# lhoyer/improving_segmentation_with_selfsupervised_depth

Hardware: AMD Instinct MI355X
Metric: train images/sec, ResNet-101 joint seg+depth @512x1024 (higher is better)
Workload: dtype f32

## Files before the change

improving_segmentation_with_selfsupervised_depth_amd/_lib.py:

```python
import ctypes
import os
from ctypes import c_int, c_long, c_float, c_void_p, c_size_t, c_uint64, c_int64, POINTER

_HERE = os.path.dirname(os.path.abspath(__file__))
LIB_PATH = os.environ.get("SEGSDE_LIB") or os.path.join(_HERE, "libsegsde_hip.so")
ABI_VERSION = 15

_LIB = None
HOST_POINTERS_OK = False


class PackJob(ctypes.Structure):
    _fields_ = [("w", c_void_p), ("fwd", c_void_p), ("dgrad", c_void_p)] + [(n, c_int) for n in (
        "O", "I", "KH", "KW", "block0", "reserved")]


class WinoJob(ctypes.Structure):
    _fields_ = [("w", c_void_p), ("u_fwd", c_void_p), ("u_dgrad", c_void_p)] + [(n, c_int) for n in ("O", "I", "block0", "reserved")]


class ConvDesc(ctypes.Structure):
    _fields_ = [(n, c_int) for n in (
        "B", "H", "W", "C0", "C1", "ld0", "ld1", "up0", "Ho", "Wo", "Cout", "ldy", "ldy2", "nsplit",
        "KH", "KW", "stride", "dil", "pad", "pad_mode", "in_div", "act", "sum2x2", "accumulate", "compute")]


P = c_void_p
_SIGS = {
    "segsde_abi_version": (c_int, []),
    "segsde_conv_compute_taken": (c_int, [POINTER(ConvDesc), c_int]),
    "segsde_split_bf16_planes": (c_int, [P, c_long, P, P, P, P]),
    "segsde_conv2d_forward": (c_int, [POINTER(ConvDesc), P, P, P, P, P, P, P]),
    "segsde_conv2d_stats_rows": (c_long, [POINTER(ConvDesc)]),
    "segsde_conv2d_forward_stats": (c_int, [POINTER(ConvDesc), P, P, P, P, P, P, P, P]),
    "segsde_conv2d_dgrad_actgrad": (c_int, [POINTER(ConvDesc), P, P, P, P, P, P, P, P, c_int, c_int, P]),
    "segsde_bn_stats_from_partials_workspace": (c_size_t, [c_int]),
    "segsde_bn_stats_from_partials": (c_int, [P, c_long, c_long, c_int, P, P, P, P, c_float, c_float, P, P, c_size_t, P]),
    "segsde_conv2d_wgrad_workspace": (c_size_t, [POINTER(ConvDesc)]),
    "segsde_conv2d_wgrad": (c_int, [POINTER(ConvDesc), P, P, P, c_int, P, P, c_size_t, P]),
# ... 5 lines not shown
    "segsde_conv2d_wgrad_winograd_workspace": (c_size_t, [POINTER(ConvDesc)]),
    "segsde_conv2d_wgrad_winograd": (c_int, [POINTER(ConvDesc), P, P, P, c_int, P, P, P, c_size_t, P]),
    "segsde_winograd_fused_ok": (c_int, [c_int, c_int, c_int, c_int, c_int]),
    "segsde_winograd_fused_stats_rows": (ctypes.c_long, [c_int, c_int, c_int]),
    "segsde_winograd_fused_pack": (c_int, [P, c_int, c_int, c_int, P, P]),
    "segsde_conv2d_winograd_fused": (c_int, [P, c_int, c_int, c_int, c_int, c_int, c_int, P, c_int, P, c_int, P, c_int, c_int, P, P]),
    "segsde_conv2d_winograd_fused2": (c_int, [P, c_int, c_int, c_int, P, c_int, c_int, c_int, c_int, c_int, c_int, P, c_int, P, c_int, P,
                                              c_int, P, P]),
    "segsde_conv2d_winograd_fused_dgrad": (c_int, [P, c_int, c_int, c_int, c_int, c_int, P, c_int, c_int, P, c_int, c_int, P, c_int, c_int, P]),
    "segsde_reflect_adjoint_borders": (c_int, [P, P, P, P, P, c_int, c_int, P]),
    "segsde_reflect_adjoint_borders_ok": (c_int, [P, c_int]),
    "segsde_reflect_adjoint_borders2": (c_int, [P, c_int, P, c_int, P, c_int, P, c_int, c_int, c_int, c_int, c_int, c_int, c_int, P]),
    "segsde_conv2d_wgrad_winograd_fused_workspace": (c_size_t, [P]),
    "segsde_conv2d_wgrad_winograd_fused": (c_int, [P, P, P, P, c_int, P, P, c_size_t, P]),
    "segsde_upfold_pack": (c_int, [P, c_int, c_int, c_int, P, P, P]),
    "segsde_conv2d_forward_upfold": (c_int, [POINTER(ConvDesc), P, P, P, P, P, P, P]),
    "segsde_conv2d_dgrad_upfold": (c_int, [POINTER(ConvDesc), P, c_int, P, P, P, P, P, c_int, P, c_int, c_int, P]),
    "segsde_conv2d_wgrad_upfold_workspace": (c_size_t, [POINTER(ConvDesc)]),
    "segsde_conv2d_wgrad_upfold": (c_int, [POINTER(ConvDesc), P, P, P, c_int, P, P, c_size_t, P]),
    "segsde_stem_pack": (c_int, [P, c_int, c_int, c_int, P, P]),
    "segsde_stem7x7_stats_rows": (c_long, [c_int, c_int, c_int, c_int, c_int]),
    "segsde_stem7x7_forward": (c_int, [P, c_int, c_int, c_int, c_int, P, c_int, P, P, P]),
    "segsde_stem7x7_wgrad_workspace": (c_size_t, [c_int, c_int, c_int, c_int, c_int]),
    "segsde_stem7x7_wgrad": (c_int, [P, c_int, c_int, c_int, c_int, P, c_int, c_int, c_int, P, P, c_size_t, P]),
    "segsde_nchw_to_nhwc_bordered": (c_int, [P, c_int, c_int, c_int, c_int, c_float, c_float, P, c_int, c_int, c_int, c_int, c_int, P]),
    "segsde_pack_weight": (c_int, [P, P, c_int, c_int, c_int, c_int, c_int, P]),
    "segsde_pack_weight_both": (c_int, [P, P, P, c_int, c_int, c_int, c_int, P]),
    "segsde_pack_weight_both_multi": (c_int, [P, c_int, c_int, P]),
    "segsde_reflect_dgrad_fix": (c_int, [P, c_int, P, P, c_int, P, c_int, c_int, c_int, c_int, c_int, c_int, c_int, P]),
    "segsde_bn_stats_workspace": (c_size_t, [c_long, c_int]),
    "segsde_bn_stats": (c_int, [P, c_int, c_long, c_int, P, P, P, P, c_float, c_float, P, P, c_size_t, P]),
    "segsde_bn_eval_stats": (c_int, [P, P, c_int, c_float, P, P, P]),
    "segsde_bn_apply": (c_int, [P, c_int, c_long, c_int, P, P, P, P, P, c_int, P, c_int, c_int, c_float, c_uint64, P]),
    "segsde_bn_backward_workspace": (c_size_t, [c_long, c_int]),
    "segsde_bn_backward": (c_int, [P, c_int, P, c_int, P, c_int, c_long, c_int, P, P, P, P, c_int, c_float, c_uint64, c_int,
                                   P, P, P, c_int, P, c_int, P, c_size_t, P]),
    "segsde_colsum_workspace": (c_size_t, [c_long, c_int]),
    "segsde_act_backward": (c_int, [P, c_int, P, c_int, c_long, c_int, c_int, P, c_int, P, P, c_size_t, P]),
    "segsde_colsum": (c_int, [P, c_int, c_long, c_int, P, P, c_size_t, P]),
    "segsde_feat_dist_workspace": (c_size_t, [c_long, c_int]),
    "segsde_feat_dist_forward": (c_int, [P, c_int, P, c_int, c_long, c_int, P, P, c_size_t, P]),
    "segsde_feat_dist_backward": (c_int, [P, c_int, P, c_int, c_long, c_int, P, P, P, c_int, P]),
    "segsde_maxpool3x3s2_forward": (c_int, [P, c_int, c_int, c_int, c_int, P, P, P]),
    "segsde_maxpool3x3s2_backward": (c_int, [P, P, c_int, c_int, c_int, c_int, P, c_int, P]),
    "segsde_upsample2x_backward": (c_int, [P, c_int, c_int, c_int, c_int, c_int, P, c_int, P]),
    "segsde_upsample2x_forward": (c_int, [P, c_int, c_int, c_int, c_int, c_int, P, c_int, P]),
    "segsde_resize_bilinear_forward": (c_int, [P, c_int, c_int, c_int, c_int, c_int, P, c_int, c_int, c_int, c_int, P]),
    "segsde_resize_bilinear_backward": (c_int, [P, c_int, c_int, c_int, c_int, c_int, P, c_int, c_int, c_int, c_int, P]),
    "segsde_global_avgpool_workspace": (c_size_t, [c_int, c_long, c_int]),
    "segsde_global_avgpool_forward": (c_int, [P, c_int, c_int, c_long, c_int, P, P, c_size_t, P]),
    "segsde_global_avgpool_backward": (c_int, [P, c_int, c_long, c_int, P, c_int, P]),
    "segsde_gate_forward": (c_int, [P, P, c_long, P, P]),
    "segsde_gate_backward": (c_int, [P, P, P, c_long, P, P, P]),
    "segsde_axpby": (c_int, [c_long, c_float, P, c_float, P, P, P]),
    "segsde_axpby_dev": (c_int, [c_long, P, P, P, P, P, P]),
    "segsde_scale_channels": (c_int, [P, c_int, c_int, c_long, c_int, P, P, c_int, P]),
    "segsde_dropout": (c_int, [P, c_int, c_long, c_int, c_float, c_uint64, P, c_int, P]),
    "segsde_copy_channels": (c_int, [P, c_int, P, c_int, c_long, c_int, P]),
    "segsde_nchw_to_nhwc": (c_int, [P, c_int, c_int, c_int, c_int, c_float, c_float, P, c_int, P]),
    "segsde_nhwc_to_nchw": (c_int, [P, c_int, c_int, c_int, c_int, c_int, P, P]),
    "segsde_pose_matrix_forward": (c_int, [P, P, c_int, c_int, c_int, P, P]),
    "segsde_pose_matrix_backward": (c_int, [P, P, P, c_int, c_int, c_int, P, P, P]),
    "segsde_warp_forward": (c_int, [P, c_int, c_int, P, P, P, P, c_int, c_int, c_int, c_float, c_float, P, P, P, P]),
    "segsde_warp_backward_workspace": (c_size_t, [c_int, c_int, c_int]),
    "segsde_warp_backward": (c_int, [P, P, c_int, c_int, P, P, P, P, c_int, c_int, c_int, c_float, c_float, P, P, P,
                                     c_size_t, P]),
    "segsde_reprojection_error_forward": (c_int, [P, P, c_int, c_int, c_int, c_int, P, c_long, P]),
# ... 74 lines not shown
```

improving_segmentation_with_selfsupervised_depth_amd/csrc/elementwise.hip:

```cpp
#include <stdlib.h>
#include "segsde_common.h"
#include <type_traits>
#include <utility>
#include <cstdlib>
#include <cstring>

namespace {

template <int VW> struct VecF { float v[VW]; };
template <int VW> __device__ __forceinline__ VecF<VW> ldv(const float* p) {
  VecF<VW> r;
  if (VW == 4) { const float4 t = *reinterpret_cast<const float4*>(p); r.v[0] = t.x; r.v[1 % VW] = t.y; r.v[2 % VW] = t.z; r.v[3 % VW] = t.w; }
  else r.v[0] = p[0];
  return r;
}
template <int VW> __device__ __forceinline__ void stv(float* p, const VecF<VW>& r) {
  if (VW == 4) *reinterpret_cast<float4*>(p) = make_float4(r.v[0], r.v[1 % VW], r.v[2 % VW], r.v[3 % VW]);
  else p[0] = r.v[0];
}

constexpr int SLAB = 64;
constexpr int RLANES = 4;

__host__ __device__ inline int red_blocks(long M) {
// ... 97 lines not shown
                                                                float momentum, float* mean, float* invstd,
                                                                float* running_mean, float* running_var, int64_t* nbt) {
  SEGSDE_SMEM;
  double* sh = reinterpret_cast<double*>(segsde_smem);
  const int c = blockIdx.x * 16 + (threadIdx.x & 15), pl = threadIdx.x >> 4;
  if (nbt && blockIdx.x == 0 && threadIdx.x == 0) nbt[0] += 1;
  double s, q;
  combine_partials(part, nb, C, c, pl, sh, s, q);
  if (pl != 0 || c >= C) return;
  const double mu = s / (double)M;
  double var = q / (double)M - mu * mu;
  if (var < 0.0) var = 0.0;
  mean[c] = (float)mu;
  invstd[c] = (float)(1.0 / sqrt(var + (double)eps));
  if (running_mean) running_mean[c] = (1.f - momentum) * running_mean[c] + momentum * (float)mu;
  if (running_var) {
    const double unb = M > 1 ? var * (double)M / (double)(M - 1) : var;
    running_var[c] = (1.f - momentum) * running_var[c] + momentum * (float)unb;
  }
}

__global__ __launch_bounds__(256) void bn_eval_stats_kernel(const float* rm, const float* rv, int C, float eps,
                                                            float* mean, float* invstd) {
  const int c = blockIdx.x * 256 + threadIdx.x;
  if (c >= C) return;
  mean[c] = rm[c];
  invstd[c] = 1.0f / sqrtf(rv[c] + eps);
}

template <int VW>
__global__ __launch_bounds__(256) void bn_apply_kernel(const float* x, int ldx, long M, int C, const float* mean,
                                                       const float* invstd, const float* gamma, const float* beta,
                                                       const float* res, int ldr, float* y, int ldy, int act,
                                                       float drop_p, uint64_t seed, int cv_shift) {
  const int CV = C / VW;
  const long total = M * CV;
  const float keep_scale = drop_p > 0.f ? 1.f / (1.f - drop_p) : 1.f;
  const long stride = (long)gridDim.x * 256;
  const bool fixed_c = cv_shift >= 0 && (stride & (long)(CV - 1)) == 0;
  VecF<VW> mu, is, ga, be;
  if (fixed_c) {
    const int c = (int)((blockIdx.x * 256L + threadIdx.x) & (long)(CV - 1)) * VW;
    mu = ldv<VW>(mean + c); is = ldv<VW>(invstd + c);
    if (gamma) { ga = ldv<VW>(gamma + c); be = ldv<VW>(beta + c); }
  }
  auto finish = [&](long m, int c, const VecF<VW>& xv, const VecF<VW>& rv) {
    VecF<VW> o;
#pragma unroll
    for (int j = 0; j < VW; ++j) {
      float t = (xv.v[j] - mu.v[j]) * is.v[j];
      if (gamma) t = t * ga.v[j] + be.v[j];
      if (res) t += rv.v[j];
      t = segsde_act(t, act);
      if (drop_p > 0.f) t = segsde_uniform01(seed, (uint64_t)(m * C + c + j)) >= drop_p ? t * keep_scale : 0.f;
      o.v[j] = t;
    }
    stv<VW>(y + m * ldy + c, o);
  };
  long e = blockIdx.x * 256L + threadIdx.x;
  for (; e < total; e += stride) {
    const long m = cv_shift >= 0 ? (e >> cv_shift) : e / CV;
    const int c = (int)(e - m * CV) * VW;
    const VecF<VW> xv = ldv<VW>(x + m * ldx + c);
    if (!fixed_c) {
      mu = ldv<VW>(mean + c); is = ldv<VW>(invstd + c);
      if (gamma) { ga = ldv<VW>(gamma + c); be = ldv<VW>(beta + c); }
    }
    VecF<VW> rv;
    if (res) rv = ldv<VW>(res + m * ldr + c);
    finish(m, c, xv, rv);
  }
}

__device__ __forceinline__ float bn_dz(float dy, float y, int act, float drop_p, uint64_t seed, uint64_t idx) {
  float g = dy;
  if (drop_p > 0.f) {
    const bool keep = segsde_uniform01(seed, idx) >= drop_p;
    if (!keep) return 0.f;
    const float ks = 1.f / (1.f - drop_p);
    g *= ks;
    y = y / ks;
  }
  return g * segsde_act_grad_from_out(y, act);
}

__device__ __forceinline__ float bn_dz_remask(float dy, float xh, float gamma, float beta, bool affine, int act) {
  if (act != SEGSDE_ACT_RELU) return dy;
  float t = xh;
  if (affine) t = t * gamma + beta;
  return t > 0.f ? dy : 0.f;
}

struct BnBwdOp {
  const float* dy; int lddy; const float* y; int ldy; const float* x; int ldx; const float* mean; const float* invstd;
  int act, C; float drop_p; uint64_t seed; const float* gamma; const float* beta;
  template <int VW> struct Ctx { VecF<VW> mu, is, ga, be; };
  template <int VW> __device__ Ctx<VW> ctx(int c) const {
    Ctx<VW> k;
    k.mu = ldv<VW>(mean + c); k.is = ldv<VW>(invstd + c);
    if (!y && gamma) { k.ga = ldv<VW>(gamma + c); k.be = ldv<VW>(beta + c); }
    return k;
  }
  template <int VW> __device__ void row(long m, int c, const Ctx<VW>& k, double* s0, double* s1) const {
    const VecF<VW> g = ldv<VW>(dy + m * lddy + c), xx = ldv<VW>(x + m * ldx + c);
    VecF<VW> yy;
    if (y) yy = ldv<VW>(y + m * ldy + c);
#pragma unroll
    for (int j = 0; j < VW; ++j) {
      const float xh = (xx.v[j] - k.mu.v[j]) * k.is.v[j];
      const float dz = y ? bn_dz(g.v[j], yy.v[j], act, drop_p, seed, (uint64_t)(m * C + c + j))
                         : bn_dz_remask(g.v[j], xh, gamma ? k.ga.v[j] : 1.f, gamma ? k.be.v[j] : 0.f, gamma != nullptr, act);
      s0[j] += (double)dz * (double)xh; s1[j] += (double)dz;
    }
  }
};

__global__ __launch_bounds__(256) void pair_finalize_kernel(const double* part, int nb, int C, float* out0, float* out1) {
  SEGSDE_SMEM;
  double* sh = reinterpret_cast<double*>(segsde_smem);
  const int c = blockIdx.x * 16 + (threadIdx.x & 15), pl = threadIdx.x >> 4;
  double a, b;
  combine_partials(part, nb, C, c, pl, sh, a, b);
  if (pl != 0 || c >= C) return;
  if (out0) out0[c] = (float)a;
  if (out1) out1[c] = (float)b;
}

template <int VW>
__global__ __launch_bounds__(256) void bn_bwd_apply_kernel(const float* dy, int lddy, const float* y, int ldy,
                                                           const float* x, int ldx, long M, int C, const float* mean,
                                                           const float* invstd, const float* gamma, const float* beta,
                                                           int act, float drop_p, uint64_t seed, int batch_stats,
                                                           const float* dgamma, const float* dbeta, float* dx, int lddx,
                                                           float* dres, int lddres, int cv_shift) {
  const int CV = C / VW;
  const long total = M * CV;
  const float invM = 1.f / (float)M;
  const bool remask = y == nullptr;
  const long stride = (long)gridDim.x * 256;
  const bool fixed_c = cv_shift >= 0 && (stride & (long)(CV - 1)) == 0;
  VecF<VW> ga, be, mu, is, dg, db;
  auto load_params = [&](int c) {
    if (dx || remask) {
      is = ldv<VW>(invstd + c);
      if (gamma) ga = ldv<VW>(gamma + c);
      if (gamma && remask) be = ldv<VW>(beta + c);
// ... 1 lines not shown
      if (batch_stats && dx) { dg = ldv<VW>(dgamma + c); db = ldv<VW>(dbeta + c); }
    }
  };
  if (fixed_c) load_params((int)((blockIdx.x * 256L + threadIdx.x) & (long)(CV - 1)) * VW);
  auto finish = [&](long m, int c, const VecF<VW>& g, const VecF<VW>& xx, const VecF<VW>& yy) {
    VecF<VW> dz, o;
#pragma unroll
    for (int j = 0; j < VW; ++j) {
      if (remask) dz.v[j] = bn_dz_remask(g.v[j], (xx.v[j] - mu.v[j]) * is.v[j], gamma ? ga.v[j] : 1.f, gamma ? be.v[j] : 0.f, gamma != nullptr, act);
      else dz.v[j] = bn_dz(g.v[j], yy.v[j], act, drop_p, seed, (uint64_t)(m * C + c + j));
      if (dx) {
        const float gm = gamma ? ga.v[j] : 1.f;
        if (batch_stats) {
          const float xh = (xx.v[j] - mu.v[j]) * is.v[j];
          o.v[j] = gm * is.v[j] * (dz.v[j] - db.v[j] * invM - xh * dg.v[j] * invM);
        } else {
          o.v[j] = gm * is.v[j] * dz.v[j];
        }
      }
    }
    if (dres) stv<VW>(dres + m * lddres + c, dz);
    if (dx) stv<VW>(dx + m * lddx + c, o);
  };
  long e = blockIdx.x * 256L + threadIdx.x;
  for (; e < total; e += stride) {
    const long m = cv_shift >= 0 ? (e >> cv_shift) : e / CV;
    const int c = (int)(e - m * CV) * VW;
    const VecF<VW> g = ldv<VW>(dy + m * lddy + c);
    VecF<VW> xx, yy;
    if (!remask) yy = ldv<VW>(y + m * ldy + c);
    if ((dx && batch_stats) || remask) xx = ldv<VW>(x + m * ldx + c);
    if (!fixed_c) load_params(c);
    finish(m, c, g, xx, yy);
  }
}

struct ActBwdOp {
  const float* dy; int lddy; const float* y; int ldy; float* dz; int lddz; int act;
  template <int VW> __device__ void row(long m, int c, double* s0, double* s1) const {
    const VecF<VW> g = ldv<VW>(dy + m * lddy + c), yy = ldv<VW>(y + m * ldy + c);
    VecF<VW> o;
#pragma unroll
    for (int j = 0; j < VW; ++j) { o.v[j] = g.v[j] * segsde_act_grad_from_out(yy.v[j], act); s0[j] += (double)o.v[j]; }
    if (dz) stv<VW>(dz + m * lddz + c, o);
  }
};
struct ColsumOp {
  const float* x; int ld;
  template <int VW> __device__ void row(long m, int c, double* s0, double* s1) const {
    const VecF<VW> t = ldv<VW>(x + m * ld + c);
#pragma unroll
    for (int j = 0; j < VW; ++j) s0[j] += (double)t.v[j];
  }
};

__global__ __launch_bounds__(256) void maxpool_fwd_kernel(const float* x, int B, int H, int W, int C, int Ho, int Wo,
                                                          float* y, uint8_t* idx) {
  const long total = (long)B * Ho * Wo * C;
  for (long e = blockIdx.x * 256L + threadIdx.x; e < total; e += (long)gridDim.x * 256) {
    const int c = (int)(e % C); long t = e / C;
    const int wo = (int)(t % Wo); t /= Wo;
    const int ho = (int)(t % Ho); const int b = (int)(t / Ho);
    float best = -INFINITY; int bi = 0; bool first = true;
    for (int kh = 0; kh < 3; ++kh) {
      const int h = 2 * ho - 1 + kh;
      if (h < 0 || h >= H) continue;
// ... 478 lines not shown
  if (!partials || !mean || !invstd || !ws) return SEGSDE_ERR_NULL;
  if (rows <= 0 || M <= 0 || C <= 0) return SEGSDE_ERR_SHAPE;
  if (ws_bytes < segsde_bn_stats_from_partials_workspace(C)) return SEGSDE_ERR_WORKSPACE;
  if (rows <= 64) {
    hipLaunchKernelGGL(bn_stats_from_partials_kernel, dim3((C + 15) / 16), dim3(256), 4096, ST(stream), partials, rows, M, C, eps,
                       momentum, mean, invstd, running_mean, running_var, num_batches_tracked);
    SEGSDE_CHECK_LAUNCH();
    return 0;
  }
  if (rows <= partials_wide_max()) {
    hipLaunchKernelGGL(bn_stats_from_partials_wide_kernel, dim3((C + 3) / 4), dim3(256), 4096, ST(stream), partials, rows, M, C, eps,
                       momentum, mean, invstd, running_mean, running_var, num_batches_tracked);
    SEGSDE_CHECK_LAUNCH();
    return 0;
  }
  const int nb = rows < PARTIALS_NB ? (int)rows : PARTIALS_NB;
  hipLaunchKernelGGL(bn_partials_reduce_kernel, dim3(nb, (C + 63) / 64), dim3(256), 4096, ST(stream), partials, rows, C, nb,
                     (double*)ws);
  SEGSDE_CHECK_LAUNCH();
  hipLaunchKernelGGL(bn_stats_finalize_kernel, dim3((C + 15) / 16), dim3(256), 4096, ST(stream), (const double*)ws, nb, M, C,
                     eps, momentum, mean, invstd, running_mean, running_var, num_batches_tracked);
  SEGSDE_CHECK_LAUNCH();
  return 0;
}

extern "C" int segsde_bn_eval_stats(const float* rm, const float* rv, int C, float eps, float* mean, float* invstd,
                                    void* stream) {
  if (!rm || !rv || !mean || !invstd) return SEGSDE_ERR_NULL;
  hipLaunchKernelGGL(bn_eval_stats_kernel, dim3((C + 255) / 256), dim3(256), 0, ST(stream), rm, rv, C, eps, mean, invstd);
  SEGSDE_CHECK_LAUNCH();
  return 0;
}

extern "C" int segsde_bn_apply(const float* x, int ldx, long M, int C, const float* mean, const float* invstd,
                               const float* gamma, const float* beta, const float* residual, int ldr, float* y, int ldy,
                               int act, float drop_p, uint64_t seed, void* stream) {
  if (!x || !mean || !invstd || !y) return SEGSDE_ERR_NULL;
  if ((gamma == nullptr) != (beta == nullptr)) return SEGSDE_ERR_NULL;
  if (M <= 0 || C <= 0 || drop_p < 0.f || drop_p >= 1.f) return SEGSDE_ERR_SHAPE;
  const bool v4 = (C % 4 == 0) && (ldx % 4 == 0) && (ldy % 4 == 0) && al16(x) && al16(y) &&
                  (!residual || ((ldr % 4 == 0) && al16(residual)));
  if (v4)
    hipLaunchKernelGGL(bn_apply_kernel<4>, dim3(ew_blocks_cv(M * C / 4, C / 4)), dim3(256), 0, ST(stream), x, ldx, M, C, mean,
                       invstd, gamma, beta, residual, ldr, y, ldy, act, drop_p, seed, pow2_shift(C / 4));
  else
    hipLaunchKernelGGL(bn_apply_kernel<1>, dim3(ew_blocks_cv(M * C, C)), dim3(256), 0, ST(stream), x, ldx, M, C, mean, invstd,
                       gamma, beta, residual, ldr, y, ldy, act, drop_p, seed, pow2_shift(C));
  SEGSDE_CHECK_LAUNCH();
  return 0;
}

extern "C" int segsde_bn_backward(const float* dy, int lddy, const float* y, int ldy, const float* x, int ldx, long M,
                                  int C, const float* mean, const float* invstd, const float* gamma, const float* beta,
                                  int act, float drop_p, uint64_t seed, int batch_stats, float* dgamma, float* dbeta,
                                  float* dx, int lddx, float* dres, int lddres, void* ws, size_t ws_bytes, void* stream) {
  if (!dy || !x || !mean || !invstd || !dgamma || !dbeta || !ws) return SEGSDE_ERR_NULL;
  if (!y) {
    if (!(act == SEGSDE_ACT_NONE || (act == SEGSDE_ACT_RELU && drop_p <= 0.f && !dres && (!gamma || beta)))) return SEGSDE_ERR_NULL;
  }
  if (M <= 0 || C <= 0) return SEGSDE_ERR_SHAPE;
  if (ws_bytes < part_bytes(M, C)) return SEGSDE_ERR_WORKSPACE;
  if (!y) ldy = ldx;
  BnBwdOp op{dy, lddy, y, ldy, x, ldx, mean, invstd, act, C, drop_p, seed, gamma, beta};
  const bool vec = (C % 4 == 0) && (ldx % 4 == 0) && (ldy % 4 == 0) && (lddy % 4 == 0) && al16p(x) && (!y || al16p(y)) && al16p(dy) &&
                   (!gamma || (al16p(gamma) && (!beta || al16p(beta)))) && al16p(mean) && al16p(invstd);
  if (int e = launch_colreduce(op, M, C, (double*)ws, vec, ST(stream))) return e;
  hipLaunchKernelGGL(pair_finalize_kernel, dim3((C + 15) / 16), dim3(256), 4096, ST(stream), (const double*)ws,
                     red_blocks(M), C, dgamma, dbeta);
  SEGSDE_CHECK_LAUNCH();
  if (dx || dres) {
    const bool v4 = vec && (!dx || ((lddx % 4 == 0) && al16p(dx))) && (!dres || ((lddres % 4 == 0) && al16p(dres))) &&
                    al16p(dgamma) && al16p(dbeta);
    if (v4)
      hipLaunchKernelGGL(bn_bwd_apply_kernel<4>, dim3(ew_blocks_cv(M * C / 4, C / 4)), dim3(256), 0, ST(stream), dy, lddy, y, ldy, x,
                         ldx, M, C, mean, invstd, gamma, beta, act, drop_p, seed, batch_stats, (const float*)dgamma,
                         (const float*)dbeta, dx, lddx, dres, lddres, pow2_shift(C / 4));
    else
      hipLaunchKernelGGL(bn_bwd_apply_kernel<1>, dim3(ew_blocks_cv(M * C, C)), dim3(256), 0, ST(stream), dy, lddy, y, ldy, x, ldx,
                         M, C, mean, invstd, gamma, beta, act, drop_p, seed, batch_stats, (const float*)dgamma,
                         (const float*)dbeta, dx, lddx, dres, lddres, pow2_shift(C));
    SEGSDE_CHECK_LAUNCH();
  }
  return 0;
}

extern "C" int segsde_act_backward(const float* dy, int lddy, const float* y, int ldy, long M, int C, int act, float* dz,
                                   int lddz, float* dbias, void* ws, size_t ws_bytes, void* stream) {
  if (!dy || !y || !ws) return SEGSDE_ERR_NULL;
  if (M <= 0 || C <= 0) return SEGSDE_ERR_SHAPE;
  if (ws_bytes < part_bytes(M, C)) return SEGSDE_ERR_WORKSPACE;
  ActBwdOp op{dy, lddy, y, ldy, dz, lddz, act};
  const bool vec = (C % 4 == 0) && (ldy % 4 == 0) && (lddy % 4 == 0) && al16p(y) && al16p(dy) &&
                   (!dz || ((lddz % 4 == 0) && al16p(dz)));
  if (int e = launch_colreduce(op, M, C, (double*)ws, vec, ST(stream))) return e;
  if (dbias) {
    hipLaunchKernelGGL(pair_finalize_kernel, dim3((C + 15) / 16), dim3(256), 4096, ST(stream), (const double*)ws,
                       red_blocks(M), C, dbias, (float*)nullptr);
    SEGSDE_CHECK_LAUNCH();
  }
  return 0;
}

extern "C" int segsde_colsum(const float* x, int ldx, long M, int C, float* out, void* ws, size_t ws_bytes, void* stream) {
  if (!x || !out || !ws) return SEGSDE_ERR_NULL;
  if (M <= 0 || C <= 0) return SEGSDE_ERR_SHAPE;
  if (ws_bytes < part_bytes(M, C)) return SEGSDE_ERR_WORKSPACE;
  ColsumOp op{x, ldx};
  const bool vec = (C % 4 == 0) && (ldx % 4 == 0) && al16p(x);
  if (int e = launch_colreduce(op, M, C, (double*)ws, vec, ST(stream))) return e;
  hipLaunchKernelGGL(pair_finalize_kernel, dim3((C + 15) / 16), dim3(256), 4096, ST(stream), (const double*)ws,
                     red_blocks(M), C, out, (float*)nullptr);
  SEGSDE_CHECK_LAUNCH();
  return 0;
// ... 188 lines not shown
```

improving_segmentation_with_selfsupervised_depth_amd/functional.py:

```python
import collections
import weakref

import torch
from torch.autograd import Function as _TorchFunction

from . import hipops as H


class Function(_TorchFunction):

    @classmethod
    def apply(cls, *args):
        return super(_TorchFunction, cls).apply(*args)


FUSIONS = {}


def _grad_dest(param):
    from . import ddp
    return ddp.grad_destination(param) if ddp._GRAD_DEST else None


def fp32_region(fn):
# ... 222 lines not shown
            if actgrad is not None and ctx.needs_input_grad[0]:
                fusion("activation_backward_in_dgrad_epilogue", bool(H.ACTGRAD_FUSED[0]))
            if not ctx.needs_input_grad[0]:
                dx0 = None
            if x1 is None or not ctx.needs_input_grad[1]:
                dx1 = None
        if ctx.needs_input_grad[2]:
            dw = H.conv_wgrad(g, x0, x1, dz, wino_v=ctx.wino_v, out=_grad_dest(weight))
            ctx.wino_v = None
        return dx0, dx1, dw, dbias, None, None, None, None, None, None, None, None, None, None


class ActGradFn(Function):

    passes = 0

    @staticmethod
    def forward(ctx, y, act, box):
        ctx.act, ctx.box = act, box
        ctx.save_for_backward(y)
        return y.view_as(y)

    @staticmethod
    def backward(ctx, dy):
        (y,) = ctx.saved_tensors
        ActGradFn.passes += 1
        fusion("activation_backward_in_dgrad_epilogue", False)
        dz, dbias = H.act_backward(_c(dy), y, ctx.act, need_dbias=bool(ctx.box.get("need_dbias")))
        if dbias is not None:
            ctx.box["dbias"] = (dz, dz._version, dbias)
        return dz, None, None


class BNActFn(Function):

    @staticmethod
    def forward(ctx, x, gamma, beta, residual, running_mean, running_var, training, momentum, eps, act, drop_p, seed,
                partials=None, grad_box=None, nbt=None):
        ctx.grad_box = grad_box
        x = _c(x)
        if training and partials is not None:
            mean, invstd = H.bn_stats_from_partials(partials, x.numel() // x.shape[-1], running_mean, running_var, momentum,
                                                    eps, update_running=running_mean is not None, num_batches_tracked=nbt)
        elif training:
            mean, invstd = H.bn_stats(x, running_mean, running_var, momentum, eps, update_running=running_mean is not None,
                                      num_batches_tracked=nbt)
        else:
            mean, invstd = H.bn_eval_stats(running_mean, running_var, eps)
        y = H.bn_apply(x, mean, invstd, gamma, beta, residual, act, drop_p, seed)
        remask = act in ("none", "relu") and residual is None and not drop_p
        ctx.cfg = (act, drop_p, seed, training, residual is not None, remask)
        ctx.beta_param = beta
        ctx.save_for_backward(x, gamma, beta if remask else None, mean, invstd, None if remask else y)
        return y

    @staticmethod
    def backward(ctx, dy):
        x, gamma, beta, mean, invstd, y = ctx.saved_tensors
        act, drop_p, seed, training, has_res, remask = ctx.cfg
        want_g = gamma is not None and ctx.needs_input_grad[1]
        bp = ctx.beta_param
        dx, dres, dgamma, dbeta = H.bn_backward(_c(dy), y, x, mean, invstd, gamma, act, drop_p, seed, batch_stats=training,
                                                need_dx=ctx.needs_input_grad[0],
                                                need_dres=has_res and ctx.needs_input_grad[3], beta=beta,
                                                dgamma_out=_grad_dest(gamma) if want_g else None,
                                                dbeta_out=_grad_dest(bp) if (want_g and bp is not None and ctx.needs_input_grad[2]) else None)
        ctx.beta_param = None
        if gamma is None or not ctx.needs_input_grad[1]:
            dgamma = dbeta = None
        if ctx.grad_box is not None and dres is not None:
            ctx.grad_box["g"] = dres
        return dx, dgamma, dbeta, dres, None, None, None, None, None, None, None, None, None, None, None


class SplitFn(Function):

    fused_count = 0

    @staticmethod
    def forward(ctx, x, box):
        ctx.box = box
        return x.view_as(x), x.view_as(x)

    @staticmethod
    def backward(ctx, g_main, g_skip):
        box = ctx.box
        fused = bool(box.get("fused")) and g_main is not None and g_skip is not None and g_main.data_ptr() == g_skip.data_ptr()
        box.clear()
        if fused:
            SplitFn.fused_count += 1
            fusion("residual_grad_accumulate", True)
            return g_main, None
        if g_main is None:
            return g_skip, None
        if g_skip is None:
            return g_main, None
        fusion("residual_grad_accumulate", False)
        return g_main + g_skip, None

# ... 420 lines not shown
```

improving_segmentation_with_selfsupervised_depth_amd/hipops.py:

```python
import ctypes
import os
import threading

import torch

from . import _lib
from ._lib import ConvDesc, check

ACT = {"none": 0, "relu": 1, "elu": 2, "sigmoid": 3}


class _Slot(threading.local):

    def __init__(self, default=None):
        self.default = default
        self.v = default

    def __getattr__(self, name):
        if name == "v":
            return self.__dict__.setdefault("v", self.__dict__.get("default"))
        raise AttributeError(name)

    def __getitem__(self, i):
        return self.v
# ... 809 lines not shown
                            _p(running_var if update_running else None), float(momentum), float(eps),
                            _p(num_batches_tracked), _p(ws), nb, _stream(x)), "bn_stats"))
    return mean, invstd


_BN_PARTIALS_WS = {}


def bn_stats_from_partials(part, M, running_mean, running_var, momentum, eps, update_running=True, num_batches_tracked=None):
    rows, _, C = part.shape
    L = _lib.lib()
    mi = torch.empty((2, C), dtype=torch.float32, device=part.device)
    mean, invstd = mi[0], mi[1]
    nb = _BN_PARTIALS_WS.get(C)
    if nb is None:
        nb = _BN_PARTIALS_WS[C] = L.segsde_bn_stats_from_partials_workspace(C)
    ws = _ws(nb, part)
    check(L.segsde_bn_stats_from_partials(_p(part), rows, M, C, _p(mean), _p(invstd),
                                          _p(running_mean if update_running else None),
                                          _p(running_var if update_running else None), float(momentum), float(eps),
                                          _p(num_batches_tracked), _p(ws), nb, _stream(part)), "bn_stats_from_partials")
    return mean, invstd


def bn_eval_stats(running_mean, running_var, eps):
    C = running_mean.numel()
    mean = torch.empty(C, dtype=torch.float32, device=running_mean.device)
    invstd = torch.empty_like(mean)
    check(_lib.lib().segsde_bn_eval_stats(_p(running_mean), _p(running_var), C, float(eps), _p(mean), _p(invstd),
                                          _stream(running_mean)), "bn_eval_stats")
    return mean, invstd


def bn_apply(x, mean, invstd, gamma, beta, residual=None, act="none", drop_p=0.0, seed=0, out=None):
    M, C, ld = _rows(x)
    y = torch.empty(x.shape, dtype=torch.float32, device=x.device) if out is None else out
    ldr = _rows(residual)[2] if residual is not None else 0
    _timed('hbm_bn_apply', (8.0 + (4.0 if residual is not None else 0.0)) * M * C, x, lambda: check(_lib.lib().segsde_bn_apply(_p(x), ld, M, C, _p(mean), _p(invstd), _p(gamma), _p(beta), _p(residual), ldr, _p(y),
                                     _rows(y)[2], ACT[act], float(drop_p), int(seed), _stream(x)), "bn_apply"))
    return y


def bn_backward(dy, y, x, mean, invstd, gamma, act="none", drop_p=0.0, seed=0, batch_stats=True, need_dx=True,
                need_dres=False, beta=None, dgamma_out=None, dbeta_out=None):
    M, C, ldx = _rows(x)
    L = _lib.lib()

    def _dst(t):
        ok = t is not None and tuple(t.shape) == (C,) and t.is_contiguous() and t.dtype == torch.float32
        return t if ok else torch.empty(C, dtype=torch.float32, device=x.device)
    dgamma, dbeta = _dst(dgamma_out), _dst(dbeta_out)
    dx = torch.empty(x.shape, dtype=torch.float32, device=x.device) if need_dx else None
    dres = torch.empty(x.shape, dtype=torch.float32, device=x.device) if need_dres else None
    nb = L.segsde_bn_backward_workspace(M, C)
    ws = _ws(nb, x)
    _timed('hbm_bn_backward', (8.0 + (4.0 if y is not None else 0.0) + (4.0 if need_dx else 0.0) + (4.0 if need_dres else 0.0)) * M * C + 8.0 * M * C, x, lambda: check(L.segsde_bn_backward(_p(_f32(dy)), _rows(dy)[2], _p(y), _rows(y)[2] if y is not None else ldx, _p(x), ldx, M, C,
                               _p(mean), _p(invstd), _p(gamma), _p(beta), ACT[act], float(drop_p), int(seed), int(batch_stats), _p(dgamma), _p(dbeta),
                               _p(dx), C, _p(dres), C, _p(ws), nb, _stream(x)), "bn_backward"))
    return dx, dres, dgamma, dbeta


def act_backward(dy, y, act, need_dbias=False, need_dz=True):
    M, C, ldy = _rows(y)
    L = _lib.lib()
    dz = torch.empty(y.shape, dtype=torch.float32, device=y.device) if need_dz else None
    dbias = torch.empty(C, dtype=torch.float32, device=y.device) if need_dbias else None
    nb = L.segsde_colsum_workspace(M, C)
    ws = _ws(nb, y)
    _timed('hbm_act_backward', (8.0 + (4.0 if need_dz else 0.0)) * M * C, y, lambda: check(L.segsde_act_backward(_p(_f32(dy)), _rows(dy)[2], _p(y), ldy, M, C, ACT[act], _p(dz), C, _p(dbias), _p(ws), nb,
                                _stream(y)), "act_backward"))
    return dz, dbias


def colsum(x):
    M, C, ld = _rows(x)
    if C == 1 and ld == 1 and M >= 4096 and M % 64 == 0:
        return colsum(x.reshape(M // 64, 64)).sum().reshape(1)
    L = _lib.lib()
    out = torch.empty(C, dtype=torch.float32, device=x.device)
    nb = L.segsde_colsum_workspace(M, C)
    ws = _ws(nb, x)
    check(L.segsde_colsum(_p(_f32(x)), ld, M, C, _p(out), _p(ws), nb, _stream(x)), "colsum")
    return out



def feat_dist_forward(a, b):
    if tuple(a.shape) != tuple(b.shape):
# ... 639 lines not shown
```

include/segsde_hip.h:

```cpp
#ifndef SEGSDE_HIP_H
#define SEGSDE_HIP_H
#include <stddef.h>
#include <stdint.h>

#ifdef __cplusplus
extern "C" {
#endif

#define SEGSDE_ABI_VERSION 15

enum { SEGSDE_ERR_NULL = -1, SEGSDE_ERR_SHAPE = -2, SEGSDE_ERR_WORKSPACE = -3, SEGSDE_ERR_UNSUPPORTED = -4 };
enum { SEGSDE_ACT_NONE = 0, SEGSDE_ACT_RELU = 1, SEGSDE_ACT_ELU = 2, SEGSDE_ACT_SIGMOID = 3 };
enum { SEGSDE_DTYPE_F32 = 0, SEGSDE_DTYPE_I64 = 1, SEGSDE_DTYPE_U8 = 2 };
enum { SEGSDE_PAD_ZERO = 0, SEGSDE_PAD_REFLECT = 1, SEGSDE_PAD_REFLECT_ADJOINT = 2 };

int segsde_abi_version(void);

typedef struct segsde_conv_desc {
  int B, H, W;
  int C0, C1;
  int ld0, ld1;
  int up0;
  int Ho, Wo, Cout;
  int ldy, ldy2, nsplit;
  int KH, KW, stride, dil, pad;
  int pad_mode;
  int in_div;
  int act;
  int sum2x2;
  int accumulate;
  int compute;
} segsde_conv_desc;

enum { SEGSDE_DIR_FORWARD = 0, SEGSDE_DIR_DGRAD = 1, SEGSDE_DIR_WGRAD = 2, SEGSDE_DIR_UPFOLD = 4 };
int segsde_conv_compute_taken(const segsde_conv_desc* d, int direction);
int segsde_split_bf16_planes(const float* x, long n, unsigned short* h, unsigned short* m, unsigned short* l, void* stream);

int segsde_conv2d_forward(const segsde_conv_desc* d, const float* x0, const float* x1, const float* wpack,
                          const float* bias, float* y, float* y2, void* stream);
long segsde_conv2d_stats_rows(const segsde_conv_desc* d);
int segsde_conv2d_forward_stats(const segsde_conv_desc* d, const float* x0, const float* x1, const float* wpack,
                                const float* bias, float* y, float* y2, double* stats, void* stream);
// ... 14 lines not shown
size_t segsde_conv2d_wgrad_upfold_workspace(const segsde_conv_desc* d);
int segsde_conv2d_wgrad_upfold(const segsde_conv_desc* d, const float* x0, const float* x1, const float* dy, int lddy,
                               float* dw_oihw, float* workspace, size_t workspace_bytes, void* stream);

int segsde_stem_pack(const float* w_oihw, int Cout, int C, int cp, float* wstem, void* stream);
long segsde_stem7x7_stats_rows(int B, int Hp, int Wp, int cp, int Cout);
int segsde_stem7x7_forward(const float* xpad, int B, int Hp, int Wp, int cp, const float* wstem, int Cout, float* y, double* stats,
                           void* stream);
size_t segsde_stem7x7_wgrad_workspace(int B, int Hp, int Wp, int cp, int Cout);
int segsde_stem7x7_wgrad(const float* xpad, int B, int Hp, int Wp, int cp, const float* dy, int lddy, int Cout, int C,
                         float* dw_oihw, float* workspace, size_t workspace_bytes, void* stream);

int segsde_pack_weight(const float* w_oihw, float* out, int O, int I, int KH, int KW, int for_dgrad, void* stream);
int segsde_pack_weight_both(const float* w_oihw, float* out_fwd, float* out_dgrad, int O, int I, int KH, int KW,
                            void* stream);
typedef struct segsde_pack_job {
  const float* w; float* fwd; float* dgrad;
  int O, I, KH, KW, block0, reserved;
} segsde_pack_job;
int segsde_pack_weight_both_multi(const segsde_pack_job* jobs_device, int njobs, int total_blocks, void* stream);

int segsde_reflect_dgrad_fix(const float* dy, int lddy, const float* wdpack, float* dx, int lddx, float* dx2, int lddx2,
                             int nsplit, int B, int H, int W, int Cin, int Cout, void* stream);

size_t segsde_bn_stats_workspace(long M, int C);
int segsde_bn_stats(const float* x, int ldx, long M, int C, float* mean, float* invstd, float* running_mean,
                    float* running_var, float momentum, float eps, int64_t* num_batches_tracked, void* workspace,
                    size_t workspace_bytes, void* stream);
int segsde_bn_eval_stats(const float* running_mean, const float* running_var, int C, float eps, float* mean,
                         float* invstd, void* stream);
int segsde_bn_apply(const float* x, int ldx, long M, int C, const float* mean, const float* invstd, const float* gamma,
                    const float* beta, const float* residual, int ldr, float* y, int ldy, int act, float drop_p,
                    uint64_t seed, void* stream);
size_t segsde_bn_stats_from_partials_workspace(int C);
int segsde_bn_stats_from_partials(const double* partials, long rows, long M, int C, float* mean, float* invstd,
                                  float* running_mean, float* running_var, float momentum, float eps,
                                  int64_t* num_batches_tracked, void* workspace, size_t workspace_bytes, void* stream);
size_t segsde_bn_backward_workspace(long M, int C);
int segsde_bn_backward(const float* dy, int lddy, const float* y, int ldy, const float* x, int ldx, long M, int C,
                       const float* mean, const float* invstd, const float* gamma, const float* beta, int act,
                       float drop_p, uint64_t seed, int batch_stats, float* dgamma, float* dbeta, float* dx, int lddx,
                       float* dres, int lddres, void* workspace, size_t workspace_bytes, void* stream);
size_t segsde_colsum_workspace(long M, int C);
int segsde_act_backward(const float* dy, int lddy, const float* y, int ldy, long M, int C, int act, float* dz, int lddz,
                        float* dbias, void* workspace, size_t workspace_bytes, void* stream);
int segsde_colsum(const float* x, int ldx, long M, int C, float* out, void* workspace, size_t workspace_bytes,
                  void* stream);

size_t segsde_feat_dist_workspace(long M, int C);
int segsde_feat_dist_forward(const float* a, int lda, const float* b, int ldb, long M, int C, float* dist, void* workspace,
                             size_t workspace_bytes, void* stream);
int segsde_feat_dist_backward(const float* a, int lda, const float* b, int ldb, long M, int C, const float* dist,
                              const float* grad, float* da, int ldda, void* stream);

int segsde_maxpool3x3s2_forward(const float* x, int B, int H, int W, int C, float* y, uint8_t* idx, void* stream);
int segsde_maxpool3x3s2_backward(const float* dy, const uint8_t* idx, int B, int H, int W, int C, float* dx, int accumulate,
                                 void* stream);
int segsde_upsample2x_backward(const float* dy, int lddy, int B, int h, int w, int C, float* dx, int lddx, void* stream);
int segsde_upsample2x_forward(const float* x, int ldx, int B, int h, int w, int C, float* y, int ldy, void* stream);
int segsde_resize_bilinear_forward(const float* x, int ldx, int B, int Hi, int Wi, int C, float* y, int ldy, int Ho, int Wo,
                                   int align_corners, void* stream);
int segsde_resize_bilinear_backward(const float* dy, int lddy, int B, int Hi, int Wi, int C, float* dx, int lddx, int Ho,
                                    int Wo, int align_corners, void* stream);
size_t segsde_global_avgpool_workspace(int B, long HW, int C);
int segsde_global_avgpool_forward(const float* x, int ldx, int B, long HW, int C, float* y, void* ws, size_t ws_bytes,
                                  void* stream);
int segsde_global_avgpool_backward(const float* dy, int B, long HW, int C, float* dx, int lddx, void* stream);
int segsde_gate_forward(const float* f, const float* a, long n, float* y, void* stream);
int segsde_gate_backward(const float* dy, const float* f, const float* a, long n, float* df, float* da, void* stream);
int segsde_axpby(long n, float alpha, const float* x, float beta, const float* y, float* out, void* stream);
int segsde_axpby_dev(long n, const float* alpha, const float* x, const float* beta, const float* y, float* out, void* stream);
int segsde_copy_channels(const float* src, int lds, float* dst, int ldd, long M, int C, void* stream);
int segsde_scale_channels(const float* x, int ldx, int B, long HW, int C, const float* scale, float* y, int ldy, void* stream);
int segsde_dropout(const float* x, int ldx, long M, int C, float p, uint64_t seed, float* y, int ldy, void* stream);
int segsde_nchw_to_nhwc(const float* x, int B, int C, int H, int W, float mean, float std, float* y, int ldy, void* stream);
// ... 138 lines not shown
```

Measured before the change: 63.77.

## Save packed ReLU bitmask for residual BN backward instead of full output

For training BN+residual+ReLU, the forward kernel now also writes a packed 4-bit-per-byte mask of positive outputs. The full fp32 output is no longer kept for backward. A new masked backward path reads the mask instead of y, computes dz once and writes it (reused as dres), then applies dx in a second pass. This cuts activation memory and the y read. In exchange it adds a dz write and read, which the old fused path may not have needed.

Result: no change. 64.31 (median of 6 runs) (+0.8%).

```diff
diff --git a/improving_segmentation_with_selfsupervised_depth_amd/_lib.py b/improving_segmentation_with_selfsupervised_depth_amd/_lib.py
--- a/improving_segmentation_with_selfsupervised_depth_amd/_lib.py
+++ b/improving_segmentation_with_selfsupervised_depth_amd/_lib.py
@@ -4,7 +4,7 @@
 
 _HERE = os.path.dirname(os.path.abspath(__file__))
 LIB_PATH = os.environ.get("SEGSDE_LIB") or os.path.join(_HERE, "libsegsde_hip.so")
-ABI_VERSION = 15
+ABI_VERSION = 16
 
 _LIB = None
 HOST_POINTERS_OK = False
@@ -76,7 +76,10 @@
     "segsde_bn_stats": (c_int, [P, c_int, c_long, c_int, P, P, P, P, c_float, c_float, P, P, c_size_t, P]),
     "segsde_bn_eval_stats": (c_int, [P, P, c_int, c_float, P, P, P]),
     "segsde_bn_apply": (c_int, [P, c_int, c_long, c_int, P, P, P, P, P, c_int, P, c_int, c_int, c_float, c_uint64, P]),
+    "segsde_bn_apply_mask": (c_int, [P, c_int, c_long, c_int, P, P, P, P, P, c_int, P, c_int, c_int, c_float, c_uint64, P, P]),
     "segsde_bn_backward_workspace": (c_size_t, [c_long, c_int]),
+    "segsde_bn_backward_masked": (c_int, [P, c_int, P, P, c_int, c_long, c_int, P, P, P, c_int, P, P, P, c_int, P, c_int, P,
+                                          c_size_t, P]),
     "segsde_bn_backward": (c_int, [P, c_int, P, c_int, P, c_int, c_long, c_int, P, P, P, P, c_int, c_float, c_uint64, c_int,
                                    P, P, P, c_int, P, c_int, P, c_size_t, P]),
     "segsde_colsum_workspace": (c_size_t, [c_long, c_int]),
diff --git a/improving_segmentation_with_selfsupervised_depth_amd/csrc/elementwise.hip b/improving_segmentation_with_selfsupervised_depth_amd/csrc/elementwise.hip
--- a/improving_segmentation_with_selfsupervised_depth_amd/csrc/elementwise.hip
+++ b/improving_segmentation_with_selfsupervised_depth_amd/csrc/elementwise.hip
@@ -153,7 +153,7 @@
 __global__ __launch_bounds__(256) void bn_apply_kernel(const float* x, int ldx, long M, int C, const float* mean,
                                                        const float* invstd, const float* gamma, const float* beta,
                                                        const float* res, int ldr, float* y, int ldy, int act,
-                                                       float drop_p, uint64_t seed, int cv_shift) {
+                                                       float drop_p, uint64_t seed, int cv_shift, uint8_t* mask) {
   const int CV = C / VW;
   const long total = M * CV;
   const float keep_scale = drop_p > 0.f ? 1.f / (1.f - drop_p) : 1.f;
@@ -165,8 +165,9 @@
     mu = ldv<VW>(mean + c); is = ldv<VW>(invstd + c);
     if (gamma) { ga = ldv<VW>(gamma + c); be = ldv<VW>(beta + c); }
   }
-  auto finish = [&](long m, int c, const VecF<VW>& xv, const VecF<VW>& rv) {
+  auto finish = [&](long e, long m, int c, const VecF<VW>& xv, const VecF<VW>& rv) {
     VecF<VW> o;
+    unsigned bits = 0;
 #pragma unroll
     for (int j = 0; j < VW; ++j) {
       float t = (xv.v[j] - mu.v[j]) * is.v[j];
@@ -175,8 +176,10 @@
       t = segsde_act(t, act);
       if (drop_p > 0.f) t = segsde_uniform01(seed, (uint64_t)(m * C + c + j)) >= drop_p ? t * keep_scale : 0.f;
       o.v[j] = t;
+      if (VW == 4 && mask) bits |= (t > 0.f ? 1u : 0u) << j;
     }
     stv<VW>(y + m * ldy + c, o);
+    if (VW == 4 && mask) mask[e] = (uint8_t)bits;
   };
   long e = blockIdx.x * 256L + threadIdx.x;
   for (; e < total; e += stride) {
@@ -189,7 +192,7 @@
     }
     VecF<VW> rv;
     if (res) rv = ldv<VW>(res + m * ldr + c);
-    finish(m, c, xv, rv);
+    finish(e, m, c, xv, rv);
   }
 }
 
@@ -233,6 +236,30 @@
                          : bn_dz_remask(g.v[j], xh, gamma ? k.ga.v[j] : 1.f, gamma ? k.be.v[j] : 0.f, gamma != nullptr, act);
       s0[j] += (double)dz * (double)xh; s1[j] += (double)dz;
     }
+  }
+};
+
+struct BnBwdMaskOp {
+  const float* dy; int lddy; const uint8_t* mask; int CQ; const float* x; int ldx; const float* mean; const float* invstd;
+  float* dz; int lddz;
+  template <int VW> struct Ctx { VecF<VW> mu, is; };
+  template <int VW> __device__ Ctx<VW> ctx(int c) const {
+    Ctx<VW> k;
+    k.mu = ldv<VW>(mean + c); k.is = ldv<VW>(invstd + c);
+    return k;
+  }
+  template <int VW> __device__ void row(long m, int c, const Ctx<VW>& k, double* s0, double* s1) const {
+    const VecF<VW> g = ldv<VW>(dy + m * lddy + c), xx = ldv<VW>(x + m * ldx + c);
+    const unsigned bits = mask[m * CQ + (c >> 2)];
+    VecF<VW> o;
+#pragma unroll
+    for (int j = 0; j < VW; ++j) {
+      const float xh = (xx.v[j] - k.mu.v[j]) * k.is.v[j];
+      const float dzv = g.v[j] * ((bits >> ((c + j) & 3)) & 1u ? 1.f : 0.f);
+      s0[j] += (double)dzv * (double)xh; s1[j] += (double)dzv;
+      o.v[j] = dzv;
+    }
+    stv<VW>(dz + m * lddz + c, o);
   }
 };
 
@@ -300,6 +327,44 @@
     if ((dx && batch_stats) || remask) xx = ldv<VW>(x + m * ldx + c);
     if (!fixed_c) load_params(c);
     finish(m, c, g, xx, yy);
+  }
+}
+
+template <int VW>
+__global__ __launch_bounds__(256) void bn_bwd_apply_dz_kernel(const float* dz, int lddz, const float* x, int ldx, long M, int C,
+                                                              const float* mean, const float* invstd, const float* gamma,
+                                                              int batch_stats, const float* dgamma, const float* dbeta, float* dx,
+                                                              int lddx, int cv_shift) {
+  const int CV = C / VW;
+  const long total = M * CV;
+  const float invM = 1.f / (float)M;
+  const long stride = (long)gridDim.x * 256;
+  const bool fixed_c = cv_shift >= 0 && (stride & (long)(CV - 1)) == 0;
+  VecF<VW> ga, mu, is, dg, db;
+  auto load_params = [&](int c) {
+    is = ldv<VW>(invstd + c);
+    if (gamma) ga = ldv<VW>(gamma + c);
+    if (batch_stats) { mu = ldv<VW>(mean + c); dg = ldv<VW>(dgamma + c); db = ldv<VW>(dbeta + c); }
+  };
+  if (fixed_c) load_params((int)((blockIdx.x * 256L + threadIdx.x) & (long)(CV - 1)) * VW);
+  for (long e = blockIdx.x * 256L + threadIdx.x; e < total; e += stride) {
+    const long m = cv_shift >= 0 ? (e >> cv_shift) : e / CV;
+    const int c = (int)(e - m * CV) * VW;
+    const VecF<VW> d = ldv<VW>(dz + m * lddz + c);
+    VecF<VW> xx, o;
+    if (batch_stats) xx = ldv<VW>(x + m * ldx + c);
+    if (!fixed_c) load_params(c);
+#pragma unroll
+    for (int j = 0; j < VW; ++j) {
+      const float gm = gamma ? ga.v[j] : 1.f;
+      if (batch_stats) {
+        const float xh = (xx.v[j] - mu.v[j]) * is.v[j];
+        o.v[j] = gm * is.v[j] * (d.v[j] - db.v[j] * invM - xh * dg.v[j] * invM);
+      } else {
+        o.v[j] = gm * is.v[j] * d.v[j];
+      }
+    }
+    stv<VW>(dx + m * lddx + c, o);
   }
 }
 
@@ -844,22 +909,29 @@
   return 0;
 }
 
-extern "C" int segsde_bn_apply(const float* x, int ldx, long M, int C, const float* mean, const float* invstd,
-                               const float* gamma, const float* beta, const float* residual, int ldr, float* y, int ldy,
-                               int act, float drop_p, uint64_t seed, void* stream) {
+extern "C" int segsde_bn_apply_mask(const float* x, int ldx, long M, int C, const float* mean, const float* invstd,
+                                    const float* gamma, const float* beta, const float* residual, int ldr, float* y, int ldy,
+                                    int act, float drop_p, uint64_t seed, uint8_t* mask, void* stream) {
   if (!x || !mean || !invstd || !y) return SEGSDE_ERR_NULL;
   if ((gamma == nullptr) != (beta == nullptr)) return SEGSDE_ERR_NULL;
   if (M <= 0 || C <= 0 || drop_p < 0.f || drop_p >= 1.f) return SEGSDE_ERR_SHAPE;
   const bool v4 = (C % 4 == 0) && (ldx % 4 == 0) && (ldy % 4 == 0) && al16(x) && al16(y) &&
                   (!residual || ((ldr % 4 == 0) && al16(residual)));
+  if (mask && !(v4 && act == SEGSDE_ACT_RELU && drop_p <= 0.f)) return SEGSDE_ERR_UNSUPPORTED;
   if (v4)
     hipLaunchKernelGGL(bn_apply_kernel<4>, dim3(ew_blocks_cv(M * C / 4, C / 4)), dim3(256), 0, ST(stream), x, ldx, M, C, mean,
-                       invstd, gamma, beta, residual, ldr, y, ldy, act, drop_p, seed, pow2_shift(C / 4));
+                       invstd, gamma, beta, residual, ldr, y, ldy, act, drop_p, seed, pow2_shift(C / 4), mask);
   else
     hipLaunchKernelGGL(bn_apply_kernel<1>, dim3(ew_blocks_cv(M * C, C)), dim3(256), 0, ST(stream), x, ldx, M, C, mean, invstd,
-                       gamma, beta, residual, ldr, y, ldy, act, drop_p, seed, pow2_shift(C));
-  SEGSDE_CHECK_LAUNCH();
-  return 0;
+                       gamma, beta, residual, ldr, y, ldy, act, drop_p, seed, pow2_shift(C), (uint8_t*)nullptr);
+  SEGSDE_CHECK_LAUNCH();
+  return 0;
+}
+
+extern "C" int segsde_bn_apply(const float* x, int ldx, long M, int C, const float* mean, const float* invstd,
+                               const float* gamma, const float* beta, const float* residual, int ldr, float* y, int ldy,
+                               int act, float drop_p, uint64_t seed, void* stream) {
+  return segsde_bn_apply_mask(x, ldx, M, C, mean, invstd, gamma, beta, residual, ldr, y, ldy, act, drop_p, seed, nullptr, stream);
 }
 
 extern "C" int segsde_bn_backward(const float* dy, int lddy, const float* y, int ldy, const float* x, int ldx, long M,
@@ -891,6 +963,35 @@
       hipLaunchKernelGGL(bn_bwd_apply_kernel<1>, dim3(ew_blocks_cv(M * C, C)), dim3(256), 0, ST(stream), dy, lddy, y, ldy, x, ldx,
                          M, C, mean, invstd, gamma, beta, act, drop_p, seed, batch_stats, (const float*)dgamma,
                          (const float*)dbeta, dx, lddx, dres, lddres, pow2_shift(C));
+    SEGSDE_CHECK_LAUNCH();
+  }
+  return 0;
+}
+
+extern "C" int segsde_bn_backward_masked(const float* dy, int lddy, const uint8_t* mask, const float* x, int ldx, long M, int C,
+                                         const float* mean, const float* invstd, const float* gamma, int batch_stats,
+                                         float* dgamma, float* dbeta, float* dx, int lddx, float* dz, int lddz, void* ws,
+                                         size_t ws_bytes, void* stream) {
+  if (!dy || !mask || !x || !mean || !invstd || !dgamma || !dbeta || !dz || !ws) return SEGSDE_ERR_NULL;
+  if (M <= 0 || C <= 0 || C % 4 != 0 || lddy < C || ldx < C || lddz < C || (dx && lddx < C)) return SEGSDE_ERR_SHAPE;
+  if (ws_bytes < part_bytes(M, C)) return SEGSDE_ERR_WORKSPACE;
+  BnBwdMaskOp op{dy, lddy, mask, C / 4, x, ldx, mean, invstd, dz, lddz};
+  const bool vec = (ldx % 4 == 0) && (lddy % 4 == 0) && (lddz % 4 == 0) && al16p(x) && al16p(dy) && al16p(dz) && al16p(mean) &&
+                   al16p(invstd);
+  if (int e = launch_colreduce(op, M, C, (double*)ws, vec, ST(stream))) return e;
+  hipLaunchKernelGGL(pair_finalize_kernel, dim3((C + 15) / 16), dim3(256), 4096, ST(stream), (const double*)ws,
+                     red_blocks(M), C, dgamma, dbeta);
+  SEGSDE_CHECK_LAUNCH();
+  if (dx) {
+    const bool v4 = vec && (lddx % 4 == 0) && al16p(dx) && (!gamma || al16p(gamma)) && al16p(dgamma) && al16p(dbeta);
+    if (v4)
+      hipLaunchKernelGGL(bn_bwd_apply_dz_kernel<4>, dim3(ew_blocks_cv(M * C / 4, C / 4)), dim3(256), 0, ST(stream), (const float*)dz,
+                         lddz, x, ldx, M, C, mean, invstd, gamma, batch_stats, (const float*)dgamma, (const float*)dbeta, dx, lddx,
+                         pow2_shift(C / 4));
+    else
+      hipLaunchKernelGGL(bn_bwd_apply_dz_kernel<1>, dim3(ew_blocks_cv(M * C, C)), dim3(256), 0, ST(stream), (const float*)dz, lddz,
+                         x, ldx, M, C, mean, invstd, gamma, batch_stats, (const float*)dgamma, (const float*)dbeta, dx, lddx,
+                         pow2_shift(C));
     SEGSDE_CHECK_LAUNCH();
   }
   return 0;
diff --git a/improving_segmentation_with_selfsupervised_depth_amd/functional.py b/improving_segmentation_with_selfsupervised_depth_amd/functional.py
--- a/improving_segmentation_with_selfsupervised_depth_amd/functional.py
+++ b/improving_segmentation_with_selfsupervised_depth_amd/functional.py
@@ -278,6 +278,9 @@
         return dz, None, None
 
 
+BN_MASK_BWD = [__import__("os").environ.get("SEGSDE_BN_MASK_BWD", "1") != "0"]
+
+
 class BNActFn(Function):
 
     @staticmethod
@@ -293,16 +296,23 @@
                                       num_batches_tracked=nbt)
         else:
             mean, invstd = H.bn_eval_stats(running_mean, running_var, eps)
-        y = H.bn_apply(x, mean, invstd, gamma, beta, residual, act, drop_p, seed)
         remask = act in ("none", "relu") and residual is None and not drop_p
+        mask = None
+        if training and residual is not None and act == "relu" and not drop_p:
+            use_mask = BN_MASK_BWD[0] and H.bn_mask_ok(x, residual, act, drop_p)
+            fusion("bn_backward_from_mask", use_mask)
+            if use_mask:
+                y, mask = H.bn_apply(x, mean, invstd, gamma, beta, residual, act, drop_p, seed, want_mask=True)
+        if mask is None:
+            y = H.bn_apply(x, mean, invstd, gamma, beta, residual, act, drop_p, seed)
         ctx.cfg = (act, drop_p, seed, training, residual is not None, remask)
         ctx.beta_param = beta
-        ctx.save_for_backward(x, gamma, beta if remask else None, mean, invstd, None if remask else y)
+        ctx.save_for_backward(x, gamma, beta if remask else None, mean, invstd, None if (remask or mask is not None) else y, mask)
         return y
 
     @staticmethod
     def backward(ctx, dy):
-        x, gamma, beta, mean, invstd, y = ctx.saved_tensors
+        x, gamma, beta, mean, invstd, y, mask = ctx.saved_tensors
         act, drop_p, seed, training, has_res, remask = ctx.cfg
         want_g = gamma is not None and ctx.needs_input_grad[1]
         bp = ctx.beta_param
@@ -310,7 +320,8 @@
                                                 need_dx=ctx.needs_input_grad[0],
                                                 need_dres=has_res and ctx.needs_input_grad[3], beta=beta,
                                                 dgamma_out=_grad_dest(gamma) if want_g else None,
-                                                dbeta_out=_grad_dest(bp) if (want_g and bp is not None and ctx.needs_input_grad[2]) else None)
+                                                dbeta_out=_grad_dest(bp) if (want_g and bp is not None and ctx.needs_input_grad[2]) else None,
+                                                mask=mask)
         ctx.beta_param = None
         if gamma is None or not ctx.needs_input_grad[1]:
             dgamma = dbeta = None
diff --git a/improving_segmentation_with_selfsupervised_depth_amd/hipops.py b/improving_segmentation_with_selfsupervised_depth_amd/hipops.py
--- a/improving_segmentation_with_selfsupervised_depth_amd/hipops.py
+++ b/improving_segmentation_with_selfsupervised_depth_amd/hipops.py
@@ -865,17 +865,26 @@
     return mean, invstd
 
 
-def bn_apply(x, mean, invstd, gamma, beta, residual=None, act="none", drop_p=0.0, seed=0, out=None):
+def bn_mask_ok(x, residual, act, drop_p):
+    if act != "relu" or drop_p or x.dtype != torch.float32:
+        return False
+    M, C, ld = _rows(x)
+    ts = [(x, ld)] + ([(residual, _rows(residual)[2])] if residual is not None else [])
+    return C % 4 == 0 and all(l % 4 == 0 and t.data_ptr() % 16 == 0 for t, l in ts)
+
+
+def bn_apply(x, mean, invstd, gamma, beta, residual=None, act="none", drop_p=0.0, seed=0, out=None, want_mask=False):
     M, C, ld = _rows(x)
     y = torch.empty(x.shape, dtype=torch.float32, device=x.device) if out is None else out
     ldr = _rows(residual)[2] if residual is not None else 0
-    _timed('hbm_bn_apply', (8.0 + (4.0 if residual is not None else 0.0)) * M * C, x, lambda: check(_lib.lib().segsde_bn_apply(_p(x), ld, M, C, _p(mean), _p(invstd), _p(gamma), _p(beta), _p(residual), ldr, _p(y),
-                                     _rows(y)[2], ACT[act], float(drop_p), int(seed), _stream(x)), "bn_apply"))
-    return y
+    mask = torch.empty((M, C // 4), dtype=torch.uint8, device=x.device) if want_mask else None
+    _timed('hbm_bn_apply', (8.0 + (4.0 if residual is not None else 0.0) + (0.25 if want_mask else 0.0)) * M * C, x, lambda: check(_lib.lib().segsde_bn_apply_mask(_p(x), ld, M, C, _p(mean), _p(invstd), _p(gamma), _p(beta), _p(residual), ldr, _p(y),
+                                     _rows(y)[2], ACT[act], float(drop_p), int(seed), _p(mask), _stream(x)), "bn_apply"))
+    return (y, mask) if want_mask else y
 
 
 def bn_backward(dy, y, x, mean, invstd, gamma, act="none", drop_p=0.0, seed=0, batch_stats=True, need_dx=True,
-                need_dres=False, beta=None, dgamma_out=None, dbeta_out=None):
+                need_dres=False, beta=None, dgamma_out=None, dbeta_out=None, mask=None):
     M, C, ldx = _rows(x)
     L = _lib.lib()
 
@@ -887,6 +896,14 @@
     dres = torch.empty(x.shape, dtype=torch.float32, device=x.device) if need_dres else None
     nb = L.segsde_bn_backward_workspace(M, C)
     ws = _ws(nb, x)
+    if mask is not None:
+        if act != "relu" or drop_p:
+            raise ValueError("bn_backward: the packed mask is the mask of a ReLU without dropout")
+        dz = dres if need_dres else torch.empty(x.shape, dtype=torch.float32, device=x.device)
+        _timed('hbm_bn_backward', (12.25 + (12.0 if need_dx else 0.0)) * M * C, x, lambda: check(L.segsde_bn_backward_masked(
+            _p(_f32(dy)), _rows(dy)[2], _p(mask), _p(x), ldx, M, C, _p(mean), _p(invstd), _p(gamma), int(batch_stats), _p(dgamma),
+            _p(dbeta), _p(dx), C, _p(dz), C, _p(ws), nb, _stream(x)), "bn_backward_masked"))
+        return dx, dres, dgamma, dbeta
     _timed('hbm_bn_backward', (8.0 + (4.0 if y is not None else 0.0) + (4.0 if need_dx else 0.0) + (4.0 if need_dres else 0.0)) * M * C + 8.0 * M * C, x, lambda: check(L.segsde_bn_backward(_p(_f32(dy)), _rows(dy)[2], _p(y), _rows(y)[2] if y is not None else ldx, _p(x), ldx, M, C,
                                _p(mean), _p(invstd), _p(gamma), _p(beta), ACT[act], float(drop_p), int(seed), int(batch_stats), _p(dgamma), _p(dbeta),
                                _p(dx), C, _p(dres), C, _p(ws), nb, _stream(x)), "bn_backward"))
diff --git a/include/segsde_hip.h b/include/segsde_hip.h
--- a/include/segsde_hip.h
+++ b/include/segsde_hip.h
@@ -7,7 +7,7 @@
 extern "C" {
 #endif
 
-#define SEGSDE_ABI_VERSION 15
+#define SEGSDE_ABI_VERSION 16
 
 enum { SEGSDE_ERR_NULL = -1, SEGSDE_ERR_SHAPE = -2, SEGSDE_ERR_WORKSPACE = -3, SEGSDE_ERR_UNSUPPORTED = -4 };
 enum { SEGSDE_ACT_NONE = 0, SEGSDE_ACT_RELU = 1, SEGSDE_ACT_ELU = 2, SEGSDE_ACT_SIGMOID = 3 };
@@ -88,6 +88,9 @@
 int segsde_bn_apply(const float* x, int ldx, long M, int C, const float* mean, const float* invstd, const float* gamma,
                     const float* beta, const float* residual, int ldr, float* y, int ldy, int act, float drop_p,
                     uint64_t seed, void* stream);
+int segsde_bn_apply_mask(const float* x, int ldx, long M, int C, const float* mean, const float* invstd, const float* gamma,
+                         const float* beta, const float* residual, int ldr, float* y, int ldy, int act, float drop_p,
+                         uint64_t seed, uint8_t* mask, void* stream);
 size_t segsde_bn_stats_from_partials_workspace(int C);
 int segsde_bn_stats_from_partials(const double* partials, long rows, long M, int C, float* mean, float* invstd,
                                   float* running_mean, float* running_var, float momentum, float eps,
@@ -97,6 +100,10 @@
                        const float* mean, const float* invstd, const float* gamma, const float* beta, int act,
                        float drop_p, uint64_t seed, int batch_stats, float* dgamma, float* dbeta, float* dx, int lddx,
                        float* dres, int lddres, void* workspace, size_t workspace_bytes, void* stream);
+int segsde_bn_backward_masked(const float* dy, int lddy, const uint8_t* mask, const float* x, int ldx, long M, int C,
+                              const float* mean, const float* invstd, const float* gamma, int batch_stats, float* dgamma,
+                              float* dbeta, float* dx, int lddx, float* dz, int lddz, void* workspace, size_t workspace_bytes,
+                              void* stream);
 size_t segsde_colsum_workspace(long M, int C);
 int segsde_act_backward(const float* dy, int lddy, const float* y, int ldy, long M, int C, int act, float* dz, int lddz,
                         float* dbias, void* workspace, size_t workspace_bytes, void* stream);
```
